# TencentARC/ViT-Lens

Measured on AMD Instinct MI355X. Metric: modality-pairs/sec (ViT-L, 224^2 patches), higher is better.
Workload: dtype bf16; 1 GPU; C3: ViT-L Lens(depth)->ViT + image + text tri-modal InfoNCE TRAINING step (fwd+bwd+AdamW), batch 1024/GPU in micro-batches of 256, first 4 blocks + adapter trainable; global_batch=1024, residual_dtype=bf16, accumulate=fp32, parallelism=dp1, gemm_cfg=-1, via=step, text_tower_operands=fp16, layernorm=folded into the GEMMs (frozen blocks), frozen_towers=second HIP stream beside the trainable tower's forward, backward=two halves of the micro-batches on two HIP streams

## Files before the change

### include/vitlens_hip.h

```cpp
#ifndef VITLENS_HIP_H
#define VITLENS_HIP_H

#include <stdint.h>

#ifdef __cplusplus
extern "C" {
#endif

#ifndef __HIP_PLATFORM_AMD__
typedef struct ihipStream_t* hipStream_t;
#endif

#define VL_EPI_BF16 0
#define VL_EPI_F32 1
#define VL_EPI_RES_F32 2
#define VL_EPI_RES_BF16 3
#define VL_EPI_GEGLU 5
#define VL_EPI_DGELU 6
#define VL_EPI_DGEGLU 7
#define VL_ACT_NONE 0
#define VL_ACT_GELU 1
#define VL_ACT_RELU 2
#define VL_ACT_GELU_DSAVE 4
#define VL_ACT_QGELU 5
// ... 116 lines not shown
int vl_layernorm_bwd(const void* dy, int dy_dtype, long dy_stride, const void* x, int x_dtype, long x_stride,
                     const float* mean, const float* rstd, const float* w, const float* dres, float* dx,
                     void* dx_bf16, long dx_stride, int rows, int D, hipStream_t stream);
int vl_layernorm_bwd_g(const void* dy, int dy_dtype, long dy_stride, const void* x, int x_dtype, long x_stride,
                       const float* mean, const float* rstd, const float* w, const void* dres, void* dx, int g_dtype,
                       void* dx_bf16, long dx_stride, int rows, int D, hipStream_t stream);
int vl_layernorm_bwd_sres(const void* dy, int dy_dtype, long dy_stride, const void* x, int x_dtype, long x_stride,
                          const float* mean, const float* rstd, const float* w, const void* dres, int dres_every,
                          long dres_stride, void* dx, int g_dtype, void* dx_bf16, long dx_stride, int rows, int D,
                          hipStream_t stream);
long vl_colreduce_ws_floats(int rows, int cols, int planes);
int vl_layernorm_bwd_params(const void* dy, int dy_dtype, long dy_stride, const void* x, int x_dtype, long x_stride,
                            const float* mean, const float* rstd, float* dw, float* db, int rows, int D,
                            float* ws, hipStream_t stream);
int vl_colsum(const void* a, int a_dtype, long lda, float* out, int rows, int cols, float scale, float* ws, hipStream_t stream);
int vl_gelu_bf16(const void* u, void* y, long n, hipStream_t stream);
int vl_geglu_bf16(const void* h, void* y, long rows, int n_out, hipStream_t stream);
int vl_attn_bwd_bf16(const void* q, const void* k, const void* v, const void* dO, const void* o, const long* strides,
                     const float* lse, float* delta, void* dq, void* dk, void* dv, long ld_dq, long ld_dkv,
                     int B, int H, int Lq, int Lk, int dh, float qscale, int causal, float scale, hipStream_t stream);
int vl_attn_bwd_fused_supported(int Lq, int Lk, int dh, int causal);
int vl_attn_bwd_fused_bf16(const void* q, const void* k, const void* v, const void* dO, const void* o, const long* strides,
                           const float* lse, void* dq, void* dk, void* dv, long ld_dq, long ld_dkv, int B, int H, int L, int dh,
                           float qscale, float scale, hipStream_t stream);
int vl_attn_fwd_q1(const void* q, const void* k, const void* v, const long* strides, void* out, long ld_out, float* lse,
                   int B, int H, int L, int dh, int qrow, float qscale, hipStream_t stream);
int vl_attn_bwd_q1(const void* q, const void* k, const void* v, const long* strides, const void* dO, long ld_do,
                   const void* o, long ld_o, const float* lse, void* dq, void* dk, void* dv, long ld_dq, long ld_dkv,
                   int B, int H, int L, int dh, int qrow, float qscale, float scale, hipStream_t stream);
int vl_attn_fwd_drop_bf16(const void* q, const void* k, const void* v, const long* strides, void* out, float* lse, int B, int H,
// ... 123 lines not shown
```

### vit-lens_amd/csrc/vl_bwd.hip

```cpp
#include "vl_common.h"
#include "vitlens_hip.h"

namespace {

__device__ __forceinline__ float ld1(const float* p) { return *p; }
__device__ __forceinline__ float ld1(const bf16_t* p) { return bf2f(*p); }

__device__ __forceinline__ void ld4(const float* p, float (&v)[4]) {
  const f32x4 t = *(const f32x4*)p; v[0] = t[0]; v[1] = t[1]; v[2] = t[2]; v[3] = t[3];
}
__device__ __forceinline__ void ld4(const bf16_t* p, float (&v)[4]) {
  const u32x2 t = *(const u32x2*)p;
  v[0] = bf2f((bf16_t)(t[0] & 0xffff)); v[1] = bf2f((bf16_t)(t[0] >> 16));
  v[2] = bf2f((bf16_t)(t[1] & 0xffff)); v[3] = bf2f((bf16_t)(t[1] >> 16));
}
__device__ __forceinline__ void st4(float* p, const float (&v)[4]) { f32x4 t = {v[0], v[1], v[2], v[3]}; *(f32x4*)p = t; }
__device__ __forceinline__ void st4(bf16_t* p, const float (&v)[4]) {
  u32x2 t; t[0] = pack2bf(v[0], v[1]); t[1] = pack2bf(v[2], v[3]); *(u32x2*)p = t;
}

struct LnBwdP {
  const void* dy; const void* x; const float* mean; const float* rstd; const float* w;
  const void* dres;
  void* dx; bf16_t* dxb;
// ... 52 lines not shown
    for (int e = lane; e < D; e += 64) {
      const float g = ld1(dy + e) * p.w[e];
      const float xh = (ld1(x + e) - mu) * rs;
      s1 += g; s2 = fmaf(g, xh, s2);
    }
    s1 = wave_sum(s1) / (float)D; s2 = wave_sum(s2) / (float)D;
    for (int e = lane; e < D; e += 64) {
      const float g = ld1(dy + e) * p.w[e];
      const float xh = (ld1(x + e) - mu) * rs;
      float v = rs * (g - s1 - xh * s2);
      if (dres) v += ld1(dres + e);
      if (dx) { if constexpr (sizeof(TG) == 4) dx[e] = v; else dx[e] = f2bf(v); }
      if (dxb) dxb[e] = f2bf(v);
    }
  }
}

__global__ void __launch_bounds__(256) gelu_kernel(const bf16_t* u, bf16_t* y, long n) {
  for (long i = ((long)blockIdx.x * 256 + threadIdx.x) * 8; i < n; i += (long)gridDim.x * 256 * 8) {
    const u32x4 v = *(const u32x4*)(u + i);
    u32x4 o;
#pragma unroll
    for (int e = 0; e < 4; ++e)
      o[e] = pack2bf(gelu_erf(bf2f((bf16_t)(v[e] & 0xffff))), gelu_erf(bf2f((bf16_t)(v[e] >> 16))));
    *(u32x4*)(y + i) = o;
  }
}

__global__ void __launch_bounds__(256) geglu_kernel(const bf16_t* h, bf16_t* y, long n) {
  for (long i = ((long)blockIdx.x * 256 + threadIdx.x) * 4; i < n; i += (long)gridDim.x * 256 * 4) {
// ... 226 lines not shown
                                     const float* mean, const float* rstd, const float* w, const void* dres, int dres_every,
                                     long dres_stride, void* dx, int g_dtype, void* dx_bf16, long dx_stride, int rows, int D,
                                     hipStream_t stream) {
  if (!dres || !dx || dres_every < 1) return vl_set_error("vl_layernorm_bwd_sres: dres, dx and dres_every >= 1 are required");
  if (dres == dx) return vl_set_error("vl_layernorm_bwd_sres: dres must not alias dx");
  return ln_bwd_run(dy, dy_dtype, dy_stride, x, x_dtype, x_stride, mean, rstd, w, dres, dres_every, dres_stride, dx, g_dtype, dx_bf16,
                    dx_stride, rows, D, stream);
}

extern "C" int vl_layernorm_bwd(const void* dy, int dy_dtype, long dy_stride, const void* x, int x_dtype, long x_stride,
                                const float* mean, const float* rstd, const float* w, const float* dres, float* dx,
                                void* dx_bf16, long dx_stride, int rows, int D, hipStream_t stream) {
  return vl_layernorm_bwd_g(dy, dy_dtype, dy_stride, x, x_dtype, x_stride, mean, rstd, w, dres, dx, VL_F32, dx_bf16, dx_stride, rows, D, stream);
}

extern "C" int vl_gelu_bf16(const void* u, void* y, long n, hipStream_t stream) {
  if (n <= 0) return 0;
  if (n & 7) return vl_set_error("vl_gelu_bf16: n must be a multiple of 8");
  hipLaunchKernelGGL(gelu_kernel, dim3(grid_for(n / 8)), dim3(256), 0, stream, (const bf16_t*)u, (bf16_t*)y, n);
  VL_HIP_OK(hipGetLastError());
  return 0;
}

extern "C" int vl_geglu_bf16(const void* h, void* y, long rows, int n_out, hipStream_t stream) {
  const long n = rows * n_out;
  if (n <= 0) return 0;
  if (n_out & 3) return vl_set_error("vl_geglu_bf16: n_out must be a multiple of 4");
  hipLaunchKernelGGL(geglu_kernel, dim3(grid_for(n / 4)), dim3(256), 0, stream, (const bf16_t*)h, (bf16_t*)y, n);
  VL_HIP_OK(hipGetLastError());
  return 0;
// ... 71 lines not shown
```

### vit-lens_amd/csrc/vl_colreduce.hip

```cpp
#include "vl_common.h"
#include "vitlens_hip.h"

namespace {

template <int V, typename T>
__device__ __forceinline__ void ldv(const T* p, float (&f)[V]) {
  constexpr bool kF32 = sizeof(T) == 4;
  static_assert(V == 1 || (kF32 ? V == 4 : V == 4 || V == 8), "no load of this width");
  if constexpr (V == 1) {
    if constexpr (kF32) f[0] = *p; else f[0] = bf2f(*p);
  } else if constexpr (kF32) {
    const f32x4 v = *(const f32x4*)p;
#pragma unroll
    for (int e = 0; e < 4; ++e) f[e] = v[e];
  } else {
    typedef __attribute__((ext_vector_type(V / 2))) unsigned int words_t;
    const words_t v = *(const words_t*)p;
#pragma unroll
    for (int e = 0; e < V / 2; ++e) { f[2 * e] = bf2f((bf16_t)(v[e] & 0xffff)); f[2 * e + 1] = bf2f((bf16_t)(v[e] >> 16)); }
  }
}

template <int V, int NR, int U, bool LN, typename TA, typename TX>
__global__ void __launch_bounds__(256) colreduce_kernel(const TA* a, long lda, const TX* x, long xs, const float* mean,
// ... 89 lines not shown
  }
  if (ry) {
#pragma unroll
    for (int e = 0; e < 4; ++e) { sh[ry - 1][cx][e] = a[e]; sh[ry - 1][cx][4 + e] = b[e]; }
  }
  __syncthreads();
  if (ry == 0 && j < D) {
#pragma unroll
    for (int e = 0; e < 4; ++e) {
      ws[((long)blockIdx.y * 2) * D + j + e] = (a[e] + sh[0][cx][e]) + (sh[1][cx][e] + sh[2][cx][e]);
      ws[((long)blockIdx.y * 2 + 1) * D + j + e] = (b[e] + sh[0][cx][4 + e]) + (sh[1][cx][4 + e] + sh[2][cx][4 + e]);
    }
  }
}

__global__ void __launch_bounds__(1024) slab_finalize_kernel(const float* ws, int nslab, int K, int D, float scale, float* out0, float* out1) {
  __shared__ float sh[16][64];
  const int jl = threadIdx.x & 63, g = threadIdx.x >> 6;
  const int j = blockIdx.x * 64 + jl, k = blockIdx.y;
  float s = 0.f;
  if (j < D)
    for (int t = g; t < nslab; t += 16) s += ws[((long)t * K + k) * D + j];
  sh[g][jl] = s;
  __syncthreads();
  if (g == 0 && j < D) {
    float a[16];
#pragma unroll
    for (int i = 0; i < 16; ++i) a[i] = sh[i][jl];
#pragma unroll
    for (int w = 8; w > 0; w >>= 1)
#pragma unroll
      for (int i = 0; i < w; ++i) a[i] += a[i + w];
    float* o = k == 0 ? out0 : out1;
    o[j] += a[0] * scale;
  }
}

}

extern "C" int vl_set_error(const char* msg);
#define VL_HIP_OK(e) do { hipError_t _e = (e); if (_e != hipSuccess) return vl_set_error(hipGetErrorString(_e)); } while (0)

static const int kSlabRows = 256;
extern "C" long vl_colreduce_ws_floats(int rows, int cols, int planes) {
  return (long)((rows + kSlabRows - 1) / kSlabRows) * planes * cols;
}

template <typename T>
// ... 14 lines not shown
                             int rows, int cols, float scale, float* out0, float* out1, hipStream_t stream) {
  const int nslab = (rows + kSlabRows - 1) / kSlabRows;
  bool vec = false;
  if constexpr (V > 1) {
    vec = vec_ok<TA>(V, a, lda, cols) && (!LN || vec_ok<TX>(V, x, xs, cols));
    if constexpr (LN && V == 4) {
      if (vec)
        hipLaunchKernelGGL(ln_bwd_params4_bf16_f32_kernel, dim3((cols + 255) / 256, nslab), dim3(256), 0, stream, (const bf16_t*)a, lda,
                           (const float*)x, xs, mean, rstd, ws, rows, cols, kSlabRows);
    } else if (vec) {
      stage1_launch<V, 4, LN ? 2 : 4, LN, TA, TX>(a, lda, x, xs, mean, rstd, ws, rows, cols, nslab, stream);
    }
  }
  if (!vec) stage1_launch<1, 1, 1, LN, TA, TX>(a, lda, x, xs, mean, rstd, ws, rows, cols, nslab, stream);
  hipLaunchKernelGGL(slab_finalize_kernel, dim3((cols + 63) / 64, LN ? 2 : 1), dim3(1024), 0, stream, ws, nslab, LN ? 2 : 1, cols,
                     scale, out0, out1);
}

extern "C" int vl_layernorm_bwd_params(const void* dy, int dy_dtype, long dy_stride, const void* x, int x_dtype, long x_stride,
                                       const float* mean, const float* rstd, float* dw, float* db, int rows, int D,
                                       float* ws, hipStream_t stream) {
  if (rows <= 0 || D <= 0) return vl_set_error("vl_layernorm_bwd_params: empty problem");
  if (!ws) return vl_set_error("vl_layernorm_bwd_params: workspace of vl_colreduce_ws_floats(rows, D, 2) floats required");
#define VL_LN_PARAMS(V, TA, TX) colreduce_launch<V, true, TA, TX>(dy, dy_stride, x, x_stride, mean, rstd, ws, rows, D, 1.0f, dw, db, stream)
  if (dy_dtype == VL_BF16 && x_dtype == VL_F32) VL_LN_PARAMS(4, bf16_t, float);
  else if (dy_dtype == VL_BF16) VL_LN_PARAMS(8, bf16_t, bf16_t);
  else if (x_dtype == VL_F32) VL_LN_PARAMS(1, float, float);
  else VL_LN_PARAMS(1, float, bf16_t);
#undef VL_LN_PARAMS
  VL_HIP_OK(hipGetLastError());
  return 0;
// ... 11 lines not shown
```

### vit-lens_amd/vitlens_hip/_lib.py

```python
import ctypes as C
import os

_HERE = os.path.dirname(os.path.abspath(__file__))
_LIB = None


class LibraryNotBuilt(ImportError):
    pass


def lib_path() -> str:
    return os.path.join(_HERE, "libvitlens_hip.so")


P, I, L, F = C.c_void_p, C.c_int, C.c_long, C.c_float

ABI_VERSION = 610

SIGNATURES = {
    "vl_version": [],
    "vl_device_info": [I, C.c_char_p, I, C.POINTER(I), C.POINTER(I), C.POINTER(L)],
    "vl_gemm_bf16": [P, P, P, P, P, I, I, I, I, I, I, F, I, I, I, P],
    "vl_gemm_splitk_accum_f32": [P, P, P, I, I, I, I, I, L, F, I, P, P],
    "vl_gemm_tn_splitk_accum_f32": [P, P, P, I, I, I, I, I, L, F, I, P, P],
# ... 57 lines not shown
    "vl_bn_stats": [P, L, I, I, P, I, P, P, P, P, F, P],
    "vl_bn_stats_local": [P, L, I, I, P, I, P, P],
    "vl_bn_stats_merge": [P, I, I, P, P, P, P, F, P, P],
    "vl_bn_bwd_reduce": [P, L, P, L, P, P, P, P, F, I, P, I, P, P, P, I, I, P],
    "vl_bn_bwd_apply": [P, L, P, L, P, P, P, P, F, I, P, P, P, L, I, I, P],
    "vl_bn_apply": [P, L, P, P, P, P, F, I, P, L, L, I, P],
    "vl_bn_bwd": [P, L, P, L, P, P, P, P, F, I, I, P, I, P, P, P, L, I, I, P],
    "vl_group_max_bwd": [P, L, P, L, P, L, P, L, L, I, I, P],
    "vl_group_sum": [P, L, P, L, L, I, I, P],
    "vl_layernorm_bwd": [P, I, L, P, I, L, P, P, P, P, P, P, L, I, I, P],
    "vl_layernorm_bwd_g": [P, I, L, P, I, L, P, P, P, P, P, I, P, L, I, I, P],
    "vl_layernorm_bwd_sres": [P, I, L, P, I, L, P, P, P, P, I, L, P, I, P, L, I, I, P],
    "vl_colreduce_ws_floats": [I, I, I],
    "vl_layernorm_bwd_params": [P, I, L, P, I, L, P, P, P, P, I, I, P, P],
    "vl_colsum": [P, I, L, P, I, I, F, P, P],
    "vl_gelu_bf16": [P, P, L, P],
    "vl_geglu_bf16": [P, P, L, I, P],
    "vl_attn_bwd_bf16": [P, P, P, P, P, P, P, P, P, P, P, L, L, I, I, I, I, I, F, I, F, P],
    "vl_attn_bwd_fused_supported": [I, I, I, I],
    "vl_attn_bwd_fused_bf16": [P, P, P, P, P, P, P, P, P, P, L, L, I, I, I, I, F, F, P],
    "vl_attn_fwd_q1": [P, P, P, P, P, L, P, I, I, I, I, I, F, P],
    "vl_attn_bwd_q1": [P, P, P, P, P, L, P, L, P, P, P, P, L, L, I, I, I, I, I, F, F, P],
    "vl_adamw_step": [P, P, P, P, L, F, F, F, F, F, I, F, P],
    "vl_sumsq_ws_floats": [],
    "vl_sumsq_f32": [P, L, P, P, P],
    "vl_adamw_multi_step": [P, I, F, F, F, F, I, F, F, P, P, P],
    "vl_clamp_scalar": [P, F, F, P],
    "vl_axpy_f32": [P, P, F, L, P],
    "vl_scale_exp_f32": [P, P, L, P, F, P],
    "vl_batch_rowsum": [P, P, I, I, I, L, L, P],
# ... 8 lines not shown
    "vl_lars_multi_step": [P, I, F, F, F, F, F, P, P, L, P],
    "vl_topk_hits": [P, L, P, I, I, I, I, P, P, P],
    "vl_eval_hits": [P, L, P, P, I, I, I, I, P, P, P, P, P, P],
    "vl_average_precision_ws_bytes": [I, I],
    "vl_average_precision": [P, L, P, L, I, I, P, P, P],
    "vl_clip_mean_normalize": [P, L, I, I, I, F, P, P],
    "vl_comm_unique_id": [P],
    "vl_comm_create": [C.POINTER(P), P, I, I],
    "vl_comm_destroy": [P],
    "vl_allgather_embed": [P, P, P, L, P],
    "vl_reducescatter_grad": [P, P, P, L, P],
    "vl_allreduce_grad": [P, P, L, P],
}


_RET = {"vl_colreduce_ws_floats": L, "vl_ce_grad_ws_floats": L, "vl_sumsq_ws_floats": L, "vl_ce_label_ws_floats": L,
        "vl_lars_ws_floats": L, "vl_average_precision_ws_bytes": L}


def load_library():
    global _LIB
    if _LIB is not None:
        return _LIB
    path = lib_path()
    if not os.path.exists(path):
        raise LibraryNotBuilt(
            f"{path} is missing: build it with `python -c 'import __graft_entry__ as g; g.build()'` "
            "or `make -C vit-lens_amd/csrc` (hipcc --offload-arch=gfx950). No CPU/eager fallback exists.")
    lib = C.CDLL(path)
    lib.vl_last_error.restype = C.c_char_p
    lib.vl_last_error.argtypes = []
# ... 22 lines not shown
```

### vit-lens_amd/vitlens_hip/ops.py

```python
import ctypes as C
import threading

import numpy as np
import torch

from ._lib import load_library, check

F32, BF16, F16 = 0, 1, 2
EPI_BF16, EPI_F32, EPI_RES_F32, EPI_RES_BF16, EPI_GEGLU, EPI_DGELU, EPI_DGEGLU = 0, 1, 2, 3, 5, 6, 7
ACT_NONE, ACT_GELU, ACT_RELU = 0, 1, 2
ACT_GELU_DSAVE = 4
ACT_QGELU = 5
ACT_QGELU_DSAVE = 6


def mlp_act(quick_gelu: bool, dsave: bool = False) -> int:
    if quick_gelu:
        return ACT_QGELU_DSAVE if dsave else ACT_QGELU
    return ACT_GELU_DSAVE if dsave else ACT_GELU
LOG2E = 1.4426950408889634

_lib = load_library()


# ... 645 lines not shown
def _ws_for(device, rows, cols, planes):
    need = int(_lib.vl_colreduce_ws_floats(rows, cols, planes))
    key = (device, torch.cuda.current_stream(device).cuda_stream, threading.get_ident())
    t = _colreduce_ws.get(key)
    if t is None or t.numel() < need:
        t = torch.empty(need, device=device, dtype=torch.float32)
        _colreduce_ws[key] = t
    return t


def layernorm_bwd_params(dy, x, mean, rstd, dw, db, rows, D, x_row_stride=None, dy_row_stride=None):
    ws = _ws_for(dy.device, rows, D, 2)
    check(_lib.vl_layernorm_bwd_params(_p(dy), _dt(dy), D if dy_row_stride is None else dy_row_stride, _p(x), _dt(x),
                                       D if x_row_stride is None else x_row_stride, _p(mean), _p(rstd), _p(dw), _p(db),
                                       rows, D, _p(ws), _stream()))


def colsum(a, out, scale=1.0):
    _chk2d(a, "a")
    ws = _ws_for(a.device, a.shape[0], a.shape[1], 1)
    check(_lib.vl_colsum(_p(a), _dt(a), a.stride(0), _p(out), a.shape[0], a.shape[1], float(scale), _p(ws), _stream()))


def geglu_bf16(h, out):
    check(_lib.vl_geglu_bf16(_p(h), _p(out), h.shape[0], h.shape[1] // 2, _stream()))
    return out


def gelu_bf16(u, out):
    check(_lib.vl_gelu_bf16(_p(u), _p(out), u.numel(), _stream()))
# ... 726 lines not shown
```

### vit-lens_amd/vitlens_hip/train.py

```python
from typing import Dict, Iterable, Optional

import torch

from . import ops
from . import engine as _engine
from .engine import VitEngine, deinterleave_geglu

BF = torch.bfloat16


class _Saved:

    def __init__(self, B, L, D, H, hidden, layers, device, res_dtype=torch.float32, keep_blocks=(), checkpoint=False):
        dh = D // H
        T = B * L
        Lp = (L + 7) // 8 * 8
        f32 = lambda *s: torch.empty(*s, device=device, dtype=torch.float32)
        bf = lambda *s: torch.empty(*s, device=device, dtype=BF)
        self.Lp = Lp
        xres = f32 if res_dtype == torch.float32 else bf

        def per_layer(make):
            if not checkpoint:
                return [make() for _ in range(layers)]
# ... 123 lines not shown
        return feat

    def _block_forward(self, S, l, B, L, write_out=True, cls_only=False, mm=0):
        e = self.eng
        def folds(k):
            return bool(_engine.LN_FOLD and S.part is not None and k < self.layers and "in_f" in e.blocks[k]
                        and k not in self.train_blocks)
        return _engine.block_forward(e.blocks[l], S.slots[l], B, L, self.D, self.H, self.causal, self.act_dsave, e.math,
                                     folds(l), folds(l + 1), cls_only=cls_only, write_out=write_out, mm=mm)

    def _dw(self, name, dy, x, bias_name=None):
        g = self.grad_buffer(name, torch.empty(dy.shape[1], x.shape[1]))
        gb = self.grad_buffer(bias_name, torch.empty(dy.shape[1])) if bias_name else None
        ops.weight_grad(dy, x, g, bias_grad=gb, narrow=False, cfg=self.eng.gemm_cfg)

    def backward(self, dfeat: torch.Tensor, on_block_done=None) -> torch.Tensor:
        e, D, H = self.eng, self.D, self.H
        B, L, tokens, has_pos2 = self.ctx
        dh = D // H
        T = L - 1 if self._drop is None else self._drop[0]
        S = self.saved(B, L)
        rows = B * L
        cfg = e.gemm_cfg
        P = self.prefix
        dfb = ops.cast_bf16(dfeat.contiguous())
        dpooled = dfb if self.proj is None else ops.gemm(dfb, self.proj, None, epi=ops.EPI_BF16, cfg=cfg)
        if self.train_proj and self.proj is not None:
            bp = (B + 63) // 64 * 64
            ops.gemm_dw(ops.transpose_to_bf16(S.pooled, ldo=bp), ops.transpose_to_bf16(dfb, ldo=bp),
                        self.grad_buffer(P + "proj", torch.empty(D, dfeat.shape[1])), cfg=cfg)
        if self.train_ln_post:
            ops.layernorm_bwd_params(dpooled, S.X[2 * self.layers], S.post_stats[0], S.post_stats[1],
                                     self.grad_buffer(P + "ln_post.weight", e.ln_post[0]),
                                     self.grad_buffer(P + "ln_post.bias", e.ln_post[1]), B, D, x_row_stride=L * D)
        if self._pruned:
            ops.layernorm_bwd(dpooled, S.X[2 * self.layers], S.post_stats[0], S.post_stats[1], e.ln_post[0], B, D,
                              dx=S.dxc, x_row_stride=L * D)
        else:
            S.dx.zero_()
            ops.layernorm_bwd(dpooled, S.X[2 * self.layers], S.post_stats[0], S.post_stats[1], e.ln_post[0], B, D,
                              dx=S.dx, x_row_stride=L * D, dx_row_stride=L * D)
        self._blocks_backward(S, B, L, on_block_done, cls_only=self._pruned)
        dxpre = torch.empty(S.dx.shape, device=S.dx.device, dtype=torch.float32)
        if self.train_ln_pre:
            ops.layernorm_bwd_params(S.dx, S.xpre, S.pre_stats[0], S.pre_stats[1], self.grad_buffer(P + "ln_pre.weight", e.ln_pre[0]),
                                     self.grad_buffer(P + "ln_pre.bias", e.ln_pre[1]), rows, D)
        ops.layernorm_bwd(S.dx, S.xpre, S.pre_stats[0], S.pre_stats[1], e.ln_pre[0], rows, D, dx=dxpre)
        if self.train_cls:
            ops.batch_rowsum(dxpre, self.grad_buffer(P + "class_embedding", e.cls).view(1, D), B, 1, D, L, 0)
        self.dxpre = dxpre
        if self._drop is not None:
            dtok = ops.scatter_rows_keep(dxpre, self._drop[1], L - 1)
            if self.train_pos:
                gpos = self.grad_buffer(P + "positional_embedding", e.pos)
                ops.batch_rowsum(dxpre, gpos[:1], B, 1, D, L, 0)
                ops.batch_rowsum(dtok, gpos[1:], B, T, D, T, 0)
            return dtok
        if self.train_pos:
            ops.batch_rowsum(dxpre, self.grad_buffer(P + "positional_embedding", e.pos), B, L, D, L, 0)
        return dxpre.view(B, L, D)[:, 1:, :].reshape(B * T, D)

# ... 7 lines not shown
        ops.layernorm_bwd(S.dhc, x1c, S.stats2c[0], S.stats2c[1], w["ln2_w"], B, D, dres=S.dxc, dx=S.dxc, x_row_stride=L * D)
        ops.gemm(S.dxc, wT["out_w"], None, out=S.dO1, epi=ops.EPI_BF16, cfg=cfg)
        ops.attn_bwd_q1(S.q[l], S.k[l], S.v[l], S.dO1, S.a1, S.lse1, S.dqkv, S.dqkv[:, D:], S.dqkv[:, 2 * D:], 3 * D, 3 * D, qrow=0)
        ops.gemm(S.dqkv, wT["in_w"], None, out=S.dh, epi=ops.EPI_BF16, cfg=cfg)
        ops.layernorm_bwd_sparse_res(S.dh, S.X[2 * l], m1, r1, w["ln1_w"], B * L, D, dres=S.dxc, dres_every=L, dx=S.dx)

    def _blocks_backward(self, S, B, L, on_block_done=None, cls_only=False):
        e, D, H = self.eng, self.D, self.H
        rows = B * L
        cfg = e.gemm_cfg
        P = self.prefix
        f32_stream = S.dx.dtype == torch.float32
        dxb_out = S.dxb if f32_stream else None
        if f32_stream:
            ops.cast_bf16(S.dx, out=S.dxb)
        for l in reversed(range(self.layers)):
            if cls_only and l == self.layers - 1:
                self._cls_block_backward(S, l, B, L)
                continue
            if self.checkpoint:
                self._block_forward(S, l, B, L, write_out=False)
            w, wT = e.blocks[l], self.wT[l]
            m1, r1, m2, r2 = S.stats[l]
            trainable = l in self.train_blocks
            bp = f"{P}transformer.resblocks.{l}."
            ops.gemm(S.dxb, wT["proj_w"], None, out=S.du, res=S.u[l], epi=ops.EPI_DGELU, act=self.act_dsave, cfg=cfg)
            if trainable:
                self._dw(bp + "mlp.c_proj.weight", S.dx, S.hidk[l], bp + "mlp.c_proj.bias")
                self._dw(bp + "mlp.c_fc.weight", S.du, S.h2[l], bp + "mlp.c_fc.bias")
            ops.gemm(S.du, wT["fc_w"], None, out=S.dh, epi=ops.EPI_BF16, cfg=cfg)
            if trainable:
                ops.layernorm_bwd_params(S.dh, S.X[2 * l + 1], m2, r2, self.grad_buffer(bp + "ln_2.weight", w["ln2_w"]),
                                         self.grad_buffer(bp + "ln_2.bias", w["ln2_b"]), rows, D)
            ops.layernorm_bwd(S.dh, S.X[2 * l + 1], m2, r2, w["ln2_w"], rows, D, dres=S.dx, dx=S.dx, dx_bf16=dxb_out)
            if trainable:
                self._dw(bp + "attn.out_proj.weight", S.dx, S.a[l], bp + "attn.out_proj.bias")
            ops.gemm(S.dxb, wT["out_w"], None, out=S.dOm, epi=ops.EPI_BF16, cfg=cfg)
            ops.attn_bwd(S.q[l], S.k[l], S.v[l], S.dO, S.av[l], S.lse[l], S.delta,
                         S.dqkv, S.dqkv[:, D:], S.dqkv[:, 2 * D:], 3 * D, 3 * D, causal=self.causal)
            if trainable:
                self._dw(bp + "attn.in_proj_weight", S.dqkv, S.h1[l], bp + "attn.in_proj_bias")
            ops.gemm(S.dqkv, wT["in_w"], None, out=S.dh, epi=ops.EPI_BF16, cfg=cfg)
            if trainable:
                ops.layernorm_bwd_params(S.dh, S.X[2 * l], m1, r1, self.grad_buffer(bp + "ln_1.weight", w["ln1_w"]),
                                         self.grad_buffer(bp + "ln_1.bias", w["ln1_b"]), rows, D)
            ops.layernorm_bwd(S.dh, S.X[2 * l], m1, r1, w["ln1_w"], rows, D, dres=S.dx, dx=S.dx, dx_bf16=dxb_out)
            if trainable and on_block_done is not None:
                on_block_done(l)


def conv_weight_grad(dtok: torch.Tensor, cols: torch.Tensor, g: torch.Tensor, gemm_cfg: int = -1):
    ops.weight_grad(ops.cast_bf16(dtok.contiguous()), cols, g, cfg=gemm_cfg)


class DepthLensTrainer:

    def __init__(self, lens_engine, unlock_first_n: int = 4, tower_kw=None):
        self.le = lens_engine
        kw = dict(train_blocks=range(unlock_first_n)) if tower_kw is None else dict(tower_kw)
        self.tower = TowerTrainer(lens_engine.vit, param_prefix="visual.", **kw)
        self.ctx = None

    @property
    def grads(self):
        return self.tower.grads

    def forward(self, x: torch.Tensor, keep=None, inv=None) -> torch.Tensor:
        le = self.le
        cols = le.cols(x)
        tok = ops.gemm(cols, le.conv_w, None, epi=ops.EPI_BF16, cfg=le.gemm_cfg)
        self.ctx = (cols, x.shape[0])
        return self.tower.forward(tok, x.shape[0], pos2=le.adapter_pos, keep=keep, inv=inv)

    def backward(self, dfeat: torch.Tensor, on_block_done=None):
        cols, B = self.ctx
        dtok = self.tower.backward(dfeat, on_block_done)
        T, D = dtok.shape[0] // B, dtok.shape[1]
        t = self.tower
        g = t.grad_buffer("visual.visual_adapter.conv1.weight_gemm", torch.empty(D, cols.shape[1]))
        conv_weight_grad(dtok, cols, g, self.le.gemm_cfg)
        gpos = t.grad_buffer("visual.visual_adapter.pos_emb", self.le.adapter_pos)
        if t._drop is not None:
            ops.batch_rowsum(dtok, gpos, B, T, D, T, 0)
        else:
            ops.batch_rowsum(t.dxpre, gpos, B, T, D, T + 1, 1)


class ImageTowerTrainer:

    def __init__(self, vit_engine, tower_kw=None, train_conv: bool = False):
        self.eng = vit_engine
        self.tower = TowerTrainer(vit_engine, param_prefix="visual.", **(tower_kw or {}))
        self.train_conv = train_conv
        self.ctx = None

    @property
# ... 432 lines not shown
```

Measured before the change: 1858 modality-pairs/sec.

## Fuse layernorm backward with parameter and bias gradient reductions in trainable blocks

Adds a row-slab layernorm backward kernel that, in one pass, computes dx (with the residual added) and per-slab column partials for dgamma, dbeta and the summed dx. The summed dx stands in for the out_proj and c_proj bias gradients, so the bias reductions in the weight-grad GEMMs are skipped. A stem kernel also fuses the ln_pre backward with the class, positional and adapter-position gradient sums, which avoids a full fp32 dxpre buffer and the separate conv cast. This removes extra full reads of dy and x from the separate params kernel and bias colsums, at the cost of more complex bookkeeping across blocks and bias gradients taken from bf16-rounded dx.

```diff
diff --git a/include/vitlens_hip.h b/include/vitlens_hip.h
--- a/include/vitlens_hip.h
+++ b/include/vitlens_hip.h
@@ -154,6 +154,14 @@
                             const float* mean, const float* rstd, float* dw, float* db, int rows, int D,
                             float* ws, hipStream_t stream);
 int vl_colsum(const void* a, int a_dtype, long lda, float* out, int rows, int cols, float scale, float* ws, hipStream_t stream);
+int vl_layernorm_bwd_partials_rows(void);
+long vl_layernorm_bwd_partials_ws_floats(int rows, int D);
+int vl_layernorm_bwd_partials(const void* dy, long dy_stride, const void* x, long x_stride, const float* mean,
+                              const float* rstd, const float* w, const void* dres, void* dx, long dx_stride, int rows,
+                              int D, float* dgamma, float* dbeta, float* dbias, float* ws, hipStream_t stream);
+int vl_layernorm_bwd_stem_batch(void);
+int vl_layernorm_bwd_stem(const void* dy, const float* x, const float* mean, const float* rstd, const float* w,
+                          void* tok_bf16, float* tok_f32, float* ws, int B, int L, int D, hipStream_t stream);
 int vl_gelu_bf16(const void* u, void* y, long n, hipStream_t stream);
 int vl_geglu_bf16(const void* h, void* y, long rows, int n_out, hipStream_t stream);
 int vl_attn_bwd_bf16(const void* q, const void* k, const void* v, const void* dO, const void* o, const long* strides,
diff --git a/vit-lens_amd/csrc/vl_bwd.hip b/vit-lens_amd/csrc/vl_bwd.hip
--- a/vit-lens_amd/csrc/vl_bwd.hip
+++ b/vit-lens_amd/csrc/vl_bwd.hip
@@ -90,6 +90,169 @@
       if (dxb) dxb[e] = f2bf(v);
     }
   }
+}
+
+template <int NCH>
+__device__ __forceinline__ void block_colsum_store(const float (&s)[NCH][4], float* sh, float* out, int wv, int lane) {
+  __syncthreads();
+  if (wv) {
+#pragma unroll
+    for (int c = 0; c < NCH; ++c) st4(sh + (wv - 1) * NCH * 256 + c * 256 + lane * 4, s[c]);
+  }
+  __syncthreads();
+  if (wv == 0) {
+#pragma unroll
+    for (int c = 0; c < NCH; ++c) {
+      float a[4], b[4], d[4], v[4];
+      ld4(sh + c * 256 + lane * 4, a); ld4(sh + NCH * 256 + c * 256 + lane * 4, b); ld4(sh + 2 * NCH * 256 + c * 256 + lane * 4, d);
+#pragma unroll
+      for (int k = 0; k < 4; ++k) v[k] = (s[c][k] + a[k]) + (b[k] + d[k]);
+      st4(out + c * 256 + lane * 4, v);
+    }
+  }
+}
+
+__device__ __forceinline__ void unpack4(const u32x2 t, float (&v)[4]) {
+  v[0] = bf2f((bf16_t)(t[0] & 0xffff)); v[1] = bf2f((bf16_t)(t[0] >> 16));
+  v[2] = bf2f((bf16_t)(t[1] & 0xffff)); v[3] = bf2f((bf16_t)(t[1] >> 16));
+}
+__device__ __forceinline__ void unpack4(const f32x4 t, float (&v)[4]) { v[0] = t[0]; v[1] = t[1]; v[2] = t[2]; v[3] = t[3]; }
+
+template <int NCH>
+struct LnRow {
+  float xh[NCH][4];
+  float s1, s2, rs;
+  template <typename XR, typename F>
+  __device__ __forceinline__ void load(const u32x2 (&dyr)[NCH], const XR (&xr)[NCH], const float* w, float mu, float rs_, int lane, int D,
+                                       F&& each) {
+#pragma clang fp contract(off)
+    rs = rs_;
+    float a1 = 0.f, a2 = 0.f;
+#pragma unroll
+    for (int c = 0; c < NCH; ++c) {
+      float g[4], ww[4];
+      unpack4(dyr[c], g); unpack4(xr[c], xh[c]); ld4(w + c * 256 + lane * 4, ww);
+#pragma unroll
+      for (int k = 0; k < 4; ++k) {
+        const float pk = g[k] * ww[k];
+        xh[c][k] = (xh[c][k] - mu) * rs;
+        a1 = a1 + pk; a2 = fmaf(pk, xh[c][k], a2);
+        each(c, k, g[k], xh[c][k]);
+      }
+    }
+    s1 = wave_sum(a1) / (float)D; s2 = wave_sum(a2) / (float)D;
+  }
+  __device__ __forceinline__ void values(int c, const u32x2 (&dyr)[NCH], const float* w, int lane, float (&v)[4]) const {
+#pragma clang fp contract(off)
+    float g[4], ww[4];
+    unpack4(dyr[c], g); ld4(w + c * 256 + lane * 4, ww);
+#pragma unroll
+    for (int k = 0; k < 4; ++k) {
+      const float t = c == 0 ? fmaf(g[k], ww[k], -s1) : g[k] * ww[k] - s1;
+      v[k] = rs * fmaf(-s2, xh[c][k], t);
+    }
+  }
+};
+
+constexpr int kLnPartRows = 88;
+template <int NCH>
+__global__ void __launch_bounds__(256) __attribute__((amdgpu_waves_per_eu(3)))
+    ln_bwd_part_kernel(const LnBwdP p, float* ws) {
+#pragma clang fp contract(off)
+  __shared__ __attribute__((aligned(16))) float sh[3 * NCH * 256];
+  const int lane = threadIdx.x & 63, wv = threadIdx.x >> 6;
+  const int r0 = blockIdx.x * kLnPartRows, r1 = min(p.rows, r0 + kLnPartRows);
+  const int D = p.D;
+  float sg[NCH][4], sb[NCH][4], sd[NCH][4];
+#pragma unroll
+  for (int c = 0; c < NCH; ++c)
+#pragma unroll
+    for (int k = 0; k < 4; ++k) { sg[c][k] = 0.f; sb[c][k] = 0.f; sd[c][k] = 0.f; }
+  struct Raw { u32x2 dy[NCH], x[NCH]; float mu, rs; };
+  auto fetch = [&](Raw& q, int row) {
+    const bf16_t* dy = (const bf16_t*)p.dy + (long)row * p.dys + lane * 4;
+    const bf16_t* x = (const bf16_t*)p.x + (long)row * p.xs + lane * 4;
+#pragma unroll
+    for (int c = 0; c < NCH; ++c) { q.dy[c] = *(const u32x2*)(dy + c * 256); q.x[c] = *(const u32x2*)(x + c * 256); }
+    q.mu = p.mean[row]; q.rs = p.rstd[row];
+  };
+  Raw cur;
+  if (r0 + wv < r1) fetch(cur, r0 + wv);
+  for (int row = r0 + wv; row < r1; row += 4) {
+    Raw nxt = cur;
+    if (row + 4 < r1) fetch(nxt, row + 4);
+    bf16_t* dx = (bf16_t*)p.dx + (long)row * p.dxs;
+    u32x2 dres[NCH];
+#pragma unroll
+    for (int c = 0; c < NCH; ++c) dres[c] = *(const u32x2*)((const bf16_t*)p.dres + (long)row * p.dxs + c * 256 + lane * 4);
+    LnRow<NCH> R;
+    R.load(cur.dy, cur.x, p.w, cur.mu, cur.rs, lane, D,
+           [&](int c, int k, float dy, float xhat) { sg[c][k] = fmaf(dy, xhat, sg[c][k]); sb[c][k] = sb[c][k] + dy; });
+#pragma unroll
+    for (int c = 0; c < NCH; ++c) {
+      const int e = c * 256 + lane * 4;
+      float v[4], r[4];
+      R.values(c, cur.dy, p.w, lane, v);
+      unpack4(dres[c], r);
+#pragma unroll
+      for (int k = 0; k < 4; ++k) v[k] = v[k] + r[k];
+      u32x2 t; t[0] = pack2bf(v[0], v[1]); t[1] = pack2bf(v[2], v[3]);
+      *(u32x2*)(dx + e) = t;
+      sd[c][0] += bf2f((bf16_t)(t[0] & 0xffff)); sd[c][1] += bf2f((bf16_t)(t[0] >> 16));
+      sd[c][2] += bf2f((bf16_t)(t[1] & 0xffff)); sd[c][3] += bf2f((bf16_t)(t[1] >> 16));
+    }
+    cur = nxt;
+  }
+  float* out = ws + (long)blockIdx.x * 3 * D;
+  block_colsum_store<NCH>(sg, sh, out, wv, lane);
+  block_colsum_store<NCH>(sb, sh, out + D, wv, lane);
+  block_colsum_store<NCH>(sd, sh, out + 2 * D, wv, lane);
+}
+
+constexpr int kStemBatch = 96;
+template <int NCH>
+__global__ void __launch_bounds__(256) ln_bwd_stem_kernel(const bf16_t* dyp, const float* xp, const float* mean, const float* rstd,
+                                                          const float* w, bf16_t* tok_bf, float* tok_f32, float* ws, int B, int L) {
+#pragma clang fp contract(off)
+  __shared__ __attribute__((aligned(16))) float sh[3 * NCH * 256];
+  constexpr int D = NCH * 256;
+  const int lane = threadIdx.x & 63, wv = threadIdx.x >> 6;
+  const int l = blockIdx.x;
+  const int b0 = blockIdx.y * kStemBatch, b1 = min(B, b0 + kStemBatch);
+  float sx[NCH][4];
+#pragma unroll
+  for (int c = 0; c < NCH; ++c)
+#pragma unroll
+    for (int k = 0; k < 4; ++k) sx[c][k] = 0.f;
+  struct Raw { u32x2 dy[NCH]; f32x4 x[NCH]; float mu, rs; };
+  auto fetch = [&](Raw& q, int b) {
+    const long row = (long)b * L + l;
+#pragma unroll
+    for (int c = 0; c < NCH; ++c) {
+      q.dy[c] = *(const u32x2*)(dyp + row * D + c * 256 + lane * 4); q.x[c] = *(const f32x4*)(xp + row * D + c * 256 + lane * 4);
+    }
+    q.mu = mean[row]; q.rs = rstd[row];
+  };
+  for (int b = b0 + wv; b < b1; b += 4) {
+    Raw cur;
+    fetch(cur, b);
+    LnRow<NCH> R;
+    R.load(cur.dy, cur.x, w, cur.mu, cur.rs, lane, D, [](int, int, float, float) {});
+    const long trow = (long)b * (L - 1) + (l - 1);
+#pragma unroll
+    for (int c = 0; c < NCH; ++c) {
+      const int e = c * 256 + lane * 4;
+      float v[4];
+      R.values(c, cur.dy, w, lane, v);
+#pragma unroll
+      for (int k = 0; k < 4; ++k) sx[c][k] = sx[c][k] + v[k];
+      if (l > 0) {
+        st4(tok_bf + trow * D + e, v);
+        if (tok_f32) st4(tok_f32 + trow * D + e, v);
+      }
+    }
+  }
+  block_colsum_store<NCH>(sx, sh, ws + ((long)blockIdx.y * L + l) * D, wv, lane);
 }
 
 __global__ void __launch_bounds__(256) gelu_kernel(const bf16_t* u, bf16_t* y, long n) {
@@ -346,6 +509,62 @@
   return vl_layernorm_bwd_g(dy, dy_dtype, dy_stride, x, x_dtype, x_stride, mean, rstd, w, dres, dx, VL_F32, dx_bf16, dx_stride, rows, D, stream);
 }
 
+void vl_slab_finalize3(const float* ws, int nslab, int D, float* out0, float* out1, float* out2, hipStream_t stream);
+
+static bool al_elems(const void* q, size_t bytes) { return (uintptr_t)q % bytes == 0; }
+
+extern "C" int vl_layernorm_bwd_partials_rows(void) { return kLnPartRows; }
+extern "C" long vl_layernorm_bwd_partials_ws_floats(int rows, int D) {
+  return (long)((rows + kLnPartRows - 1) / kLnPartRows) * 3 * D;
+}
+
+extern "C" int vl_layernorm_bwd_partials(const void* dy, long dy_stride, const void* x, long x_stride, const float* mean,
+                                         const float* rstd, const float* w, const void* dres, void* dx, long dx_stride, int rows,
+                                         int D, float* dgamma, float* dbeta, float* dbias, float* ws, hipStream_t stream) {
+  if (rows <= 0 || D <= 0) return vl_set_error("vl_layernorm_bwd_partials: empty problem");
+  if (!dy || !x || !mean || !rstd || !w || !dres || !dx || !dgamma || !dbeta || !ws)
+    return vl_set_error("vl_layernorm_bwd_partials: every operand, dgamma, dbeta and the workspace are required (dbias may be null)");
+  if ((D != 256 && D != 512 && D != 768 && D != 1024) || dy_stride % 4 || x_stride % 4 || dx_stride % 4 || !al_elems(dy, 8) ||
+      !al_elems(x, 8) || !al_elems(w, 16) || !al_elems(dres, 8) || !al_elems(dx, 8) || !al_elems(ws, 16))
+    return vl_set_error("vl_layernorm_bwd_partials: D must be 256, 512, 768 or 1024, every row stride a multiple of 4 elements "
+                        "and every base address a multiple of 4 elements (the workspace: 16 bytes)");
+  LnBwdP p{dy, x, mean, rstd, w, dres, dx, nullptr, dy_stride, x_stride, dx_stride, rows, D, 1, dx_stride};
+  const int nblk = (rows + kLnPartRows - 1) / kLnPartRows;
+  switch (D / 256) {
+    case 4: hipLaunchKernelGGL(ln_bwd_part_kernel<4>, dim3(nblk), dim3(256), 0, stream, p, ws); break;
+    case 3: hipLaunchKernelGGL(ln_bwd_part_kernel<3>, dim3(nblk), dim3(256), 0, stream, p, ws); break;
+    case 2: hipLaunchKernelGGL(ln_bwd_part_kernel<2>, dim3(nblk), dim3(256), 0, stream, p, ws); break;
+    default: hipLaunchKernelGGL(ln_bwd_part_kernel<1>, dim3(nblk), dim3(256), 0, stream, p, ws); break;
+  }
+  vl_slab_finalize3(ws, nblk, D, dgamma, dbeta, dbias, stream);
+  VL_HIP_OK(hipGetLastError());
+  return 0;
+}
+
+extern "C" int vl_layernorm_bwd_stem_batch(void) { return kStemBatch; }
+
+extern "C" int vl_layernorm_bwd_stem(const void* dy, const float* x, const float* mean, const float* rstd, const float* w,
+                                     void* tok_bf16, float* tok_f32, float* ws, int B, int L, int D, hipStream_t stream) {
+  if (B <= 0 || L < 2 || D <= 0) return vl_set_error("vl_layernorm_bwd_stem: needs B >= 1 samples of L >= 2 rows (class row + tokens)");
+  if (!dy || !x || !mean || !rstd || !w || !tok_bf16 || !ws)
+    return vl_set_error("vl_layernorm_bwd_stem: dy, x, mean, rstd, w, tok_bf16 and ws are required");
+  if ((D != 256 && D != 512 && D != 768 && D != 1024) || !al_elems(dy, 8) || !al_elems(x, 16) || !al_elems(w, 16) ||
+      !al_elems(tok_bf16, 8) || !al_elems(tok_f32, 16) || !al_elems(ws, 16))
+    return vl_set_error("vl_layernorm_bwd_stem: D must be 256, 512, 768 or 1024 and every base address a multiple of 4 elements");
+  const dim3 grid(L, (B + kStemBatch - 1) / kStemBatch);
+#define VL_STEM(N) hipLaunchKernelGGL(ln_bwd_stem_kernel<N>, grid, dim3(256), 0, stream, (const bf16_t*)dy, x, mean, rstd, w, \
+                                      (bf16_t*)tok_bf16, tok_f32, ws, B, L)
+  switch (D / 256) {
+    case 4: VL_STEM(4); break;
+    case 3: VL_STEM(3); break;
+    case 2: VL_STEM(2); break;
+    default: VL_STEM(1); break;
+  }
+#undef VL_STEM
+  VL_HIP_OK(hipGetLastError());
+  return 0;
+}
+
 extern "C" int vl_gelu_bf16(const void* u, void* y, long n, hipStream_t stream) {
   if (n <= 0) return 0;
   if (n & 7) return vl_set_error("vl_gelu_bf16: n must be a multiple of 8");
diff --git a/vit-lens_amd/csrc/vl_colreduce.hip b/vit-lens_amd/csrc/vl_colreduce.hip
--- a/vit-lens_amd/csrc/vl_colreduce.hip
+++ b/vit-lens_amd/csrc/vl_colreduce.hip
@@ -127,7 +127,8 @@
   }
 }
 
-__global__ void __launch_bounds__(1024) slab_finalize_kernel(const float* ws, int nslab, int K, int D, float scale, float* out0, float* out1) {
+__global__ void __launch_bounds__(1024) slab_finalize_kernel(const float* ws, int nslab, int K, int D, float scale, float* out0, float* out1,
+                                                             float* out2) {
   __shared__ float sh[16][64];
   const int jl = threadIdx.x & 63, g = threadIdx.x >> 6;
   const int j = blockIdx.x * 64 + jl, k = blockIdx.y;
@@ -144,7 +145,7 @@
     for (int w = 8; w > 0; w >>= 1)
 #pragma unroll
       for (int i = 0; i < w; ++i) a[i] += a[i + w];
-    float* o = k == 0 ? out0 : out1;
+    float* o = k == 0 ? out0 : (k == 1 ? out1 : out2);
     o[j] += a[0] * scale;
   }
 }
@@ -189,7 +190,11 @@
   }
   if (!vec) stage1_launch<1, 1, 1, LN, TA, TX>(a, lda, x, xs, mean, rstd, ws, rows, cols, nslab, stream);
   hipLaunchKernelGGL(slab_finalize_kernel, dim3((cols + 63) / 64, LN ? 2 : 1), dim3(1024), 0, stream, ws, nslab, LN ? 2 : 1, cols,
-                     scale, out0, out1);
+                     scale, out0, out1, nullptr);
+}
+
+void vl_slab_finalize3(const float* ws, int nslab, int D, float* out0, float* out1, float* out2, hipStream_t stream) {
+  hipLaunchKernelGGL(slab_finalize_kernel, dim3((D + 63) / 64, out2 ? 3 : 2), dim3(1024), 0, stream, ws, nslab, 3, D, 1.0f, out0, out1, out2);
 }
 
 extern "C" int vl_layernorm_bwd_params(const void* dy, int dy_dtype, long dy_stride, const void* x, int x_dtype, long x_stride,
diff --git a/vit-lens_amd/vitlens_hip/_lib.py b/vit-lens_amd/vitlens_hip/_lib.py
--- a/vit-lens_amd/vitlens_hip/_lib.py
+++ b/vit-lens_amd/vitlens_hip/_lib.py
@@ -95,6 +95,11 @@
     "vl_colreduce_ws_floats": [I, I, I],
     "vl_layernorm_bwd_params": [P, I, L, P, I, L, P, P, P, P, I, I, P, P],
     "vl_colsum": [P, I, L, P, I, I, F, P, P],
+    "vl_layernorm_bwd_partials_rows": [],
+    "vl_layernorm_bwd_partials_ws_floats": [I, I],
+    "vl_layernorm_bwd_partials": [P, L, P, L, P, P, P, P, P, L, I, I, P, P, P, P, P],
+    "vl_layernorm_bwd_stem_batch": [],
+    "vl_layernorm_bwd_stem": [P, P, P, P, P, P, P, P, I, I, I, P],
     "vl_gelu_bf16": [P, P, L, P],
     "vl_geglu_bf16": [P, P, L, I, P],
     "vl_attn_bwd_bf16": [P, P, P, P, P, P, P, P, P, P, P, L, L, I, I, I, I, I, F, I, F, P],
@@ -133,7 +138,7 @@
 }
 
 
-_RET = {"vl_colreduce_ws_floats": L, "vl_ce_grad_ws_floats": L, "vl_sumsq_ws_floats": L, "vl_ce_label_ws_floats": L,
+_RET = {"vl_colreduce_ws_floats": L, "vl_layernorm_bwd_partials_ws_floats": L,"vl_ce_grad_ws_floats": L, "vl_sumsq_ws_floats": L, "vl_ce_label_ws_floats": L,
         "vl_lars_ws_floats": L, "vl_average_precision_ws_bytes": L}
 
 
diff --git a/vit-lens_amd/vitlens_hip/ops.py b/vit-lens_amd/vitlens_hip/ops.py
--- a/vit-lens_amd/vitlens_hip/ops.py
+++ b/vit-lens_amd/vitlens_hip/ops.py
@@ -683,6 +683,60 @@
     check(_lib.vl_layernorm_bwd_params(_p(dy), _dt(dy), D if dy_row_stride is None else dy_row_stride, _p(x), _dt(x),
                                        D if x_row_stride is None else x_row_stride, _p(mean), _p(rstd), _p(dw), _p(db),
                                        rows, D, _p(ws), _stream()))
+
+
+_LN_VEC_D = (256, 512, 768, 1024)
+
+
+def _keyed_ws(cache, device, need):
+    key = (device, torch.cuda.current_stream(device).cuda_stream, threading.get_ident())
+    t = cache.get(key)
+    if t is None or t.numel() < need:
+        t = torch.empty(need, device=device, dtype=torch.float32)
+        cache[key] = t
+    return t
+
+
+_ln_part_ws = {}
+
+
+def layernorm_bwd_partials_ok(dy, x, dres, dx, D):
+    ts = (dy, x, dres, dx)
+    return (D in _LN_VEC_D and all(t is not None and t.dtype == torch.bfloat16 and t.dim() == 2 and t.stride(1) == 1
+                                   and t.stride(0) % 4 == 0 and t.data_ptr() % 8 == 0 for t in ts)
+            and dres.stride(0) == dx.stride(0))
+
+
+def layernorm_bwd_partials(dy, x, mean, rstd, w, rows, D, dres, dx, dgamma, dbeta, dbias):
+    need = int(_lib.vl_layernorm_bwd_partials_ws_floats(rows, D))
+    ws = _keyed_ws(_ln_part_ws, dy.device, need)
+    check(_lib.vl_layernorm_bwd_partials(_p(dy), dy.stride(0), _p(x), x.stride(0), _p(mean), _p(rstd), _p(w), _p(dres), _p(dx),
+                                         dx.stride(0), rows, D, _p(dgamma), _p(dbeta), _p(dbias), _p(ws), _stream()))
+
+
+def layernorm_bwd_partials_geometry(rows):
+    per = int(_lib.vl_layernorm_bwd_partials_rows())
+    return per, (rows + per - 1) // per
+
+
+def layernorm_bwd_stem_geometry(B):
+    per = int(_lib.vl_layernorm_bwd_stem_batch())
+    return per, (B + per - 1) // per
+
+
+def layernorm_bwd_stem_ok(dy, x, D, L):
+    return (D in _LN_VEC_D and L >= 2 and dy.dtype == torch.bfloat16 and x.dtype == torch.float32 and dy.is_contiguous()
+            and x.is_contiguous() and dy.data_ptr() % 8 == 0 and x.data_ptr() % 16 == 0)
+
+
+def layernorm_bwd_stem(dy, x, mean, rstd, w, B, L, D, want_f32=False):
+    T = L - 1
+    tok_bf = torch.empty(B * T, D, device=dy.device, dtype=torch.bfloat16)
+    tok_f32 = torch.empty(B * T, D, device=dy.device, dtype=torch.float32) if want_f32 else None
+    G = layernorm_bwd_stem_geometry(B)[1]
+    sums = torch.empty(G, L, D, device=dy.device, dtype=torch.float32)
+    check(_lib.vl_layernorm_bwd_stem(_p(dy), _p(x), _p(mean), _p(rstd), _p(w), _p(tok_bf), _p(tok_f32), _p(sums), B, L, D, _stream()))
+    return tok_bf, tok_f32, sums
 
 
 def colsum(a, out, scale=1.0):
diff --git a/vit-lens_amd/vitlens_hip/train.py b/vit-lens_amd/vitlens_hip/train.py
--- a/vit-lens_amd/vitlens_hip/train.py
+++ b/vit-lens_amd/vitlens_hip/train.py
@@ -7,6 +7,7 @@
 from .engine import VitEngine, deinterleave_geglu
 
 BF = torch.bfloat16
+FUSED_PARAM_GRADS = True
 
 
 class _Saved:
@@ -161,7 +162,7 @@
         gb = self.grad_buffer(bias_name, torch.empty(dy.shape[1])) if bias_name else None
         ops.weight_grad(dy, x, g, bias_grad=gb, narrow=False, cfg=self.eng.gemm_cfg)
 
-    def backward(self, dfeat: torch.Tensor, on_block_done=None) -> torch.Tensor:
+    def backward(self, dfeat: torch.Tensor, on_block_done=None, stem_tokens=False) -> torch.Tensor:
         e, D, H = self.eng, self.D, self.H
         B, L, tokens, has_pos2 = self.ctx
         dh = D // H
@@ -188,10 +189,19 @@
             ops.layernorm_bwd(dpooled, S.X[2 * self.layers], S.post_stats[0], S.post_stats[1], e.ln_post[0], B, D,
                               dx=S.dx, x_row_stride=L * D, dx_row_stride=L * D)
         self._blocks_backward(S, B, L, on_block_done, cls_only=self._pruned)
-        dxpre = torch.empty(S.dx.shape, device=S.dx.device, dtype=torch.float32)
         if self.train_ln_pre:
             ops.layernorm_bwd_params(S.dx, S.xpre, S.pre_stats[0], S.pre_stats[1], self.grad_buffer(P + "ln_pre.weight", e.ln_pre[0]),
                                      self.grad_buffer(P + "ln_pre.bias", e.ln_pre[1]), rows, D)
+        self.dxpre = self.stem_sums = None
+        if stem_tokens and FUSED_PARAM_GRADS and self._drop is None and ops.layernorm_bwd_stem_ok(S.dx, S.xpre, D, L):
+            dtok, _, sums = ops.layernorm_bwd_stem(S.dx, S.xpre, S.pre_stats[0], S.pre_stats[1], e.ln_pre[0], B, L, D)
+            if self.train_cls:
+                ops.batch_rowsum(sums, self.grad_buffer(P + "class_embedding", e.cls).view(1, D), sums.shape[0], 1, D, L, 0)
+            if self.train_pos:
+                ops.batch_rowsum(sums, self.grad_buffer(P + "positional_embedding", e.pos), sums.shape[0], L, D, L, 0)
+            self.stem_sums = sums
+            return dtok
+        dxpre = torch.empty(S.dx.shape, device=S.dx.device, dtype=torch.float32)
         ops.layernorm_bwd(S.dx, S.xpre, S.pre_stats[0], S.pre_stats[1], e.ln_pre[0], rows, D, dx=dxpre)
         if self.train_cls:
             ops.batch_rowsum(dxpre, self.grad_buffer(P + "class_embedding", e.cls).view(1, D), B, 1, D, L, 0)
@@ -229,6 +239,7 @@
         dxb_out = S.dxb if f32_stream else None
         if f32_stream:
             ops.cast_bf16(S.dx, out=S.dxb)
+        above_summed_dx = False
         for l in reversed(range(self.layers)):
             if cls_only and l == self.layers - 1:
                 self._cls_block_backward(S, l, B, L)
@@ -239,27 +250,40 @@
             m1, r1, m2, r2 = S.stats[l]
             trainable = l in self.train_blocks
             bp = f"{P}transformer.resblocks.{l}."
+            fused = trainable and FUSED_PARAM_GRADS and ops.layernorm_bwd_partials_ok(S.dh, S.X[2 * l], S.dx, S.dx, D)
             ops.gemm(S.dxb, wT["proj_w"], None, out=S.du, res=S.u[l], epi=ops.EPI_DGELU, act=self.act_dsave, cfg=cfg)
             if trainable:
-                self._dw(bp + "mlp.c_proj.weight", S.dx, S.hidk[l], bp + "mlp.c_proj.bias")
+                self._dw(bp + "mlp.c_proj.weight", S.dx, S.hidk[l], None if above_summed_dx else bp + "mlp.c_proj.bias")
                 self._dw(bp + "mlp.c_fc.weight", S.du, S.h2[l], bp + "mlp.c_fc.bias")
             ops.gemm(S.du, wT["fc_w"], None, out=S.dh, epi=ops.EPI_BF16, cfg=cfg)
+            if fused:
+                ops.layernorm_bwd_partials(S.dh, S.X[2 * l + 1], m2, r2, w["ln2_w"], rows, D, S.dx, S.dx,
+                                           self.grad_buffer(bp + "ln_2.weight", w["ln2_w"]), self.grad_buffer(bp + "ln_2.bias", w["ln2_b"]),
+                                           self.grad_buffer(bp + "attn.out_proj.bias", w["ln2_b"]))
+            else:
+                if trainable:
+                    ops.layernorm_bwd_params(S.dh, S.X[2 * l + 1], m2, r2, self.grad_buffer(bp + "ln_2.weight", w["ln2_w"]),
+                                             self.grad_buffer(bp + "ln_2.bias", w["ln2_b"]), rows, D)
+                ops.layernorm_bwd(S.dh, S.X[2 * l + 1], m2, r2, w["ln2_w"], rows, D, dres=S.dx, dx=S.dx, dx_bf16=dxb_out)
             if trainable:
-                ops.layernorm_bwd_params(S.dh, S.X[2 * l + 1], m2, r2, self.grad_buffer(bp + "ln_2.weight", w["ln2_w"]),
-                                         self.grad_buffer(bp + "ln_2.bias", w["ln2_b"]), rows, D)
-            ops.layernorm_bwd(S.dh, S.X[2 * l + 1], m2, r2, w["ln2_w"], rows, D, dres=S.dx, dx=S.dx, dx_bf16=dxb_out)
-            if trainable:
-                self._dw(bp + "attn.out_proj.weight", S.dx, S.a[l], bp + "attn.out_proj.bias")
+                self._dw(bp + "attn.out_proj.weight", S.dx, S.a[l], None if fused else bp + "attn.out_proj.bias")
             ops.gemm(S.dxb, wT["out_w"], None, out=S.dOm, epi=ops.EPI_BF16, cfg=cfg)
             ops.attn_bwd(S.q[l], S.k[l], S.v[l], S.dO, S.av[l], S.lse[l], S.delta,
                          S.dqkv, S.dqkv[:, D:], S.dqkv[:, 2 * D:], 3 * D, 3 * D, causal=self.causal)
             if trainable:
                 self._dw(bp + "attn.in_proj_weight", S.dqkv, S.h1[l], bp + "attn.in_proj_bias")
             ops.gemm(S.dqkv, wT["in_w"], None, out=S.dh, epi=ops.EPI_BF16, cfg=cfg)
-            if trainable:
-                ops.layernorm_bwd_params(S.dh, S.X[2 * l], m1, r1, self.grad_buffer(bp + "ln_1.weight", w["ln1_w"]),
-                                         self.grad_buffer(bp + "ln_1.bias", w["ln1_b"]), rows, D)
-            ops.layernorm_bwd(S.dh, S.X[2 * l], m1, r1, w["ln1_w"], rows, D, dres=S.dx, dx=S.dx, dx_bf16=dxb_out)
+            above_summed_dx = fused and (l - 1) in self.train_blocks
+            if fused:
+                below = f"{P}transformer.resblocks.{l - 1}.mlp.c_proj.bias"
+                ops.layernorm_bwd_partials(S.dh, S.X[2 * l], m1, r1, w["ln1_w"], rows, D, S.dx, S.dx,
+                                           self.grad_buffer(bp + "ln_1.weight", w["ln1_w"]), self.grad_buffer(bp + "ln_1.bias", w["ln1_b"]),
+                                           self.grad_buffer(below, w["ln1_b"]) if above_summed_dx else None)
+            else:
+                if trainable:
+                    ops.layernorm_bwd_params(S.dh, S.X[2 * l], m1, r1, self.grad_buffer(bp + "ln_1.weight", w["ln1_w"]),
+                                             self.grad_buffer(bp + "ln_1.bias", w["ln1_b"]), rows, D)
+                ops.layernorm_bwd(S.dh, S.X[2 * l], m1, r1, w["ln1_w"], rows, D, dres=S.dx, dx=S.dx, dx_bf16=dxb_out)
             if trainable and on_block_done is not None:
                 on_block_done(l)
 
@@ -289,12 +313,16 @@
 
     def backward(self, dfeat: torch.Tensor, on_block_done=None):
         cols, B = self.ctx
-        dtok = self.tower.backward(dfeat, on_block_done)
+        dtok = self.tower.backward(dfeat, on_block_done, stem_tokens=True)
         T, D = dtok.shape[0] // B, dtok.shape[1]
         t = self.tower
         g = t.grad_buffer("visual.visual_adapter.conv1.weight_gemm", torch.empty(D, cols.shape[1]))
+        gpos = t.grad_buffer("visual.visual_adapter.pos_emb", self.le.adapter_pos)
+        if t.stem_sums is not None:
+            ops.weight_grad(dtok, cols, g, cfg=self.le.gemm_cfg)
+            ops.batch_rowsum(t.stem_sums, gpos, t.stem_sums.shape[0], T, D, T + 1, 1)
+            return
         conv_weight_grad(dtok, cols, g, self.le.gemm_cfg)
-        gpos = t.grad_buffer("visual.visual_adapter.pos_emb", self.le.adapter_pos)
         if t._drop is not None:
             ops.batch_rowsum(dtok, gpos, B, T, D, T, 0)
         else:
```

Measured after the change: 1865 modality-pairs/sec, median of 6. About the same (+0.4%).
